# gusye1234/recad

Hardware: AMD Instinct MI355X
Metric: BPR train interactions/sec + full-catalog top-K scorings/sec, LightGCN ml1m dim=64 (higher is better)
Workload: dtype f32

## Files before the change

include/recad_hip.h:

```cpp
#ifndef RECAD_HIP_H
#define RECAD_HIP_H
#include <stdint.h>

#ifdef __cplusplus
extern "C" {
#endif

#define RK_ABI_VERSION 9
#define RK_OK 0
#define RK_EINVAL (-22)
#define RK_EHIP (-5)
#define RK_ENOMEM (-12)

#define RK_LOSS_PARTIALS 256

int rk_abi_version(void);
const char *rk_last_error(void);
int rk_device_info(char *name, int32_t name_len, int32_t *cu_count);

int rk_coo_to_csr(int32_t n_rows, int64_t nnz, const int64_t *coo_row, const int64_t *coo_col,
                  const float *coo_val, int32_t *rowptr , int32_t *col ,
                  float *val , void *stream);

typedef struct rk_schedule *rk_schedule_t;
// ... 139 lines not shown
    int32_t panel_rows;
    int32_t panel_ntw;
    int32_t panel_safe;
    int32_t nb, n_items, dim, K, n_targets;
    int32_t ld_scores;
    int32_t reserved[2];
    int64_t scratch_floats;
} rk_score_plan;
int rk_score_topk_plan(int32_t nb, int32_t n_items, int32_t dim, int32_t K, int32_t n_targets, const rk_score_plan *request ,
                       rk_score_plan *out);
int rk_score_topk(int32_t dim, const float *utab, int32_t nb, const int32_t *user_ids, const float *itab,
                  int32_t n_items, const float *ubias, const float *ibias, float mean,
                  const int32_t *seen_ptr, const int32_t *seen_idx, int32_t K, int32_t *top_ids,
                  float *top_scores, const int32_t *targets, int32_t n_targets, float *target_score,
                  int32_t *target_rank, const rk_score_plan *plan, float *scratch, void *stream);

int rk_mf_train_epoch(int32_t n_users, int32_t n_items, int32_t dim, float *user_emb, float *item_emb,
                      float *user_bias, float *item_bias, float mean, float *m, float *v, float *grads,
                      const int64_t *users, const int64_t *items, const int64_t *labels, int64_t n,
                      int32_t batch, int32_t adam_t0, float lr, float beta1, float beta2, float eps,
                      float *loss_partials, int32_t apply_update, float dropout, uint64_t drop_seed, void *stream);

int rk_bpr_sample(int32_t n_users, int32_t n_items, const int32_t *pos_ptr, const int32_t *pos_idx,
                  int64_t n_draws, uint64_t seed, int64_t *users, int64_t *pos, int64_t *neg, int32_t *valid,
                  void *stream);

int rk_pointwise_sample(int32_t n_users, int32_t n_items, const int32_t *train_ptr, const int32_t *train_idx,
                        int64_t n_edges, int32_t negative_ratio, uint64_t seed, int64_t *users, int64_t *items,
                        int64_t *labels, void *stream);

// ... 152 lines not shown
```

recad_amd/_lib.py:

```python
import ctypes as C
import os

import torch

_HERE = os.path.dirname(os.path.abspath(__file__))
LIB_PATH = os.path.join(_HERE, "lib", "librecad_hip.so")
RK_LOSS_PARTIALS = 256
RK_MAX_GRAPH_STEPS = 64
ABI_VERSION = 9
RK_LDS_SYNC_WORDS = 2560
RK_PCA_GRAM_BLOCKS = 256


class HipLibraryMissing(RuntimeError):
    pass


class HipCallError(RuntimeError):
    pass


class LdsInfo(C.Structure):

    _fields_ = [
# ... 137 lines not shown
    "rk_bpr_rows_ordered": [_I32, _I32, _F, _P, _P, _P, _P, _P, _P, _P, _I32, _P, _P, _P],
    "rk_lightgcn_create": [C.POINTER(LightGCNDesc), C.POINTER(_P)],
    "rk_lightgcn_destroy": [_P],
    "rk_lightgcn_sync_status": [_P, C.POINTER(_I32), _P],
    "rk_lightgcn_propagate": [_P, _P],
    "rk_lightgcn_propagate_dropout": [_P, C.c_uint64, _P],
    "rk_lightgcn_train_epoch": [_P, _P, _P, _P, _I64, _I32, _I32, _P, _I32, _I32, _P],
    "rk_lightgcn_prepare": [_P, _I64, _I32, _I32, _I32, _P],
    "rk_lightgcn_set_deterministic": [_P, _I32],
    "rk_pair_scores": [_I32, _P, _P, _P, _P, _F, _P, _P, _I64, _P, _F, C.c_uint64, _P],
    "rk_score_matrix": [_I32, _P, _I32, _P, _P, _I32, _P, _P, _F, _F, C.c_uint64, _P, _P],
    "rk_adam_step": [_I64, _P, _P, _P, _P, _I32, _F, _F, _F, _F, _P],
    "rk_adam_step_dev": [_I64, _P, _P, _P, _P, _P, _F, _F, _F, _P],
    "rk_score_topk_plan": [_I32, _I32, _I32, _I32, _I32, C.POINTER(ScorePlan), C.POINTER(ScorePlan)],
    "rk_score_topk": [_I32, _P, _I32, _P, _P, _I32, _P, _P, _F, _P, _P, _I32, _P, _P, _P, _I32, _P, _P, C.POINTER(ScorePlan), _P, _P],
    "rk_bpr_sample": [_I32, _I32, _P, _P, _I64, C.c_uint64, _P, _P, _P, _P, _P],
    "rk_pointwise_sample": [_I32, _I32, _P, _P, _I64, _I32, C.c_uint64, _P, _P, _P, _P],
    "rk_topk_rows": [_P, _I32, _I32, _P, _P, _P, _I32, _P, _P, _P, _I32, _P, _P, _P],
    "rk_hit_counts": [_P, _I64, _I32, _P, _I32, _P, _P],
    "rk_eligible_users": [_I32, _P, _P, _P, _I32, _P, _P, _P, _P],
    "rk_pred_shift": [_P, _P, _I64, _P, _P],
    "rk_users_rating": [_I32, _P, _I32, _P, _P, _I32, _P, _P],
    "rk_ncf_forward": [C.POINTER(NCFDesc), _P, _P, _P, _I32, _I64, _P, _P],
    "rk_ncf_train_epoch": [C.POINTER(NCFDesc), _P, _P, _P, _I64, _I32, _I32, _P, _I32, _P],
    "rk_mf_train_epoch": [_I32, _I32, _I32, _P, _P, _P, _P, _F, _P, _P, _P, _P, _P, _P, _I64, _I32, _I32, _F, _F, _F,
                          _F, _P, _I32, _F, C.c_uint64, _P],
    "rk_pca_transpose": [_I32, _I32, _P, _P, _P, _P, _P, _P, _P],
    "rk_pca_col_scale": [_I32, _I32, _P, _P, _P, _P, _P],
    "rk_pca_spmm": [_I32, _P, _P, _P, _P, _P, _I32, _P, _P, _P],
    "rk_pca_sq_spmv": [_I32, _I32, _P, _P, _P, _P, _I32, _I32, _P, _P, _P],
# ... 91 lines not shown
```

recad_amd/csrc/gemm.h:

```cpp
#pragma once
#include <stdlib.h>
#include <type_traits>

#include "common.h"

typedef float f32x16 __attribute__((ext_vector_type(16)));

struct GemmArgs {
    int M, N, K;
    const float *A; long long a_rs, a_cs;
    const int *a_ridx;
    int a_rmod, a_roff;
    const float *acc_init; int ld_init, init_base;
    const float *B; long long b_rs, b_cs;
    float *C; int ldc;
    const float *col_bias;
    const float *row_bias;
    float const_add;
    int relu;
    int sigmoid;
    unsigned drop_thresh24;
    float drop_scale;
    unsigned long long drop_seed;
    const float *mask; int ldmask;
    float *sk_part; long long sk_stride;
    int split_k;
};

static constexpr int kGK = 32, kGLd = kGK + 1;
template <int BT> constexpr int gemm_lds_bytes(int nbuf) { return nbuf * 2 * BT * kGLd * (int)sizeof(float); }

template <int BT> struct TileRegs { float v[BT / 8]; };

template <int BT>
__device__ __forceinline__ int tile_mode(const float *src, int n_rows, int n_k, int r0, int k0, long long rs, long long cs,
                                         bool gathered = false)
{
    const bool full = (r0 + BT <= n_rows) && (k0 + kGK <= n_k);
    if (!full) return 0;
    if (cs == 1 && (rs & 3) == 0 && ((uintptr_t)src & 15) == 0) return 1;
    if (!gathered && rs == 1 && (cs & 3) == 0 && ((uintptr_t)src & 15) == 0) return 2;
    return 0;
// ... 77 lines not shown
template <int BT, int NBUF, int MINW, bool GATHER = false, bool PLAIN = false>
static __global__ __launch_bounds__(256, MINW) void gemm_f32_kernel(const GemmArgs g, const int tiles_per_block)
{
    constexpr int kGT = BT, TA = BT / 64, WS = BT / 2;
    extern __shared__ __attribute__((aligned(16))) float smem[];
    auto tileA = [&](int buf) { return reinterpret_cast<float (*)[kGLd]>(smem + (size_t)buf * 2 * kGT * kGLd); };
    auto tileB = [&](int buf) { return reinterpret_cast<float (*)[kGLd]>(smem + (size_t)buf * 2 * kGT * kGLd + kGT * kGLd); };
    const int lane = threadIdx.x & 63, w = threadIdx.x >> 6;
    const int wr = w >> 1, wc = w & 1;
    const int gx = (g.N + kGT - 1) / kGT, gy = (g.M + kGT - 1) / kGT, nwg = gx * gy;
    int bid = blockIdx.x;
    {
        const int nb = gridDim.x, q = nb / 8, r = nb % 8, xcd = bid % 8;
        bid = (xcd < r ? xcd * (q + 1) : r * (q + 1) + (xcd - r) * q) + bid / 8;
    }
    const int t_begin = bid * tiles_per_block, t_end = min(nwg, t_begin + tiles_per_block);
    if (t_begin >= t_end) return;
    f32x16 acc[TA][TA];
#pragma unroll
    for (int i = 0; i < TA; ++i)
#pragma unroll
        for (int j = 0; j < TA; ++j)
#pragma unroll
            for (int r = 0; r < 16; ++r) acc[i][j][r] = 0.f;
    const int lr = lane & 31, lk = lane >> 5;
    const int all_chunks = (g.K + kGK - 1) / kGK;
    const int splits = g.split_k > 1 ? g.split_k : 1;
    const int per = (all_chunks + splits - 1) / splits;
    const int c_lo = (int)blockIdx.y * per, c_hi = min(all_chunks, c_lo + per);
    if (c_lo >= c_hi) return;
// ... 399 lines not shown
#define GEMM_STAMP(it, i) do { } while (0)
#endif
template <int MA, int MB, bool PLAIN = false, bool GROUPED = false>
static __global__ __launch_bounds__(256) __attribute__((amdgpu_waves_per_eu(2, 2))) void gemm_f32_wide_kernel(const GemmArgs g, const int gx, const int gy)
{
    extern __shared__ __attribute__((aligned(16))) float dsm[];
    float *sA = dsm, *sB = dsm + wide_floats<MA>();
    const int lane = threadIdx.x & 63, w = threadIdx.x >> 6, tid = threadIdx.x;
    const int wr = w >> 1, wc = w & 1;
    int bid = blockIdx.x;
    const int nb = gridDim.x;
    {
        const int q = nb / 8, r = nb % 8, xcd = bid % 8;
        bid = (xcd < r ? xcd * (q + 1) : r * (q + 1) + (xcd - r) * q) + bid / 8;
    }
    const int n_tiles = gx * gy;
    const int t_begin = (int)((long long)bid * n_tiles / nb), t_end = (int)((long long)(bid + 1) * n_tiles / nb);
    if (t_begin >= t_end) return;
    const int n_chunks = g.K / kWK, total = (t_end - t_begin) * n_chunks;
    f32x4 acc[4][4];
    const int l16 = lane & 15, lq = lane >> 4;
    long long ra[8], rb[8];
    int m0, n0, m1, n1;
    auto row_offsets = [&](int mt, int nt) {
#pragma unroll
        for (int p = 0; p < 8; ++p) {
            const int m = min(mt + p * 16 + (tid >> 4), g.M - 1);
            ra[p] = (long long)(g.a_ridx ? g.a_ridx[m] : g.a_rmod ? (m + g.a_roff) % g.a_rmod : m) * g.a_rs;
            rb[p] = (long long)min(nt + p * 16 + (tid >> 4), g.N - 1) * g.b_rs;
        }
// ... 189 lines not shown
        GEMM_STAMP(it, 6);
    }
}

inline hipError_t gemm_f32_launch(const GemmArgs &g, hipStream_t s)
{
    static RkPerDeviceOnce attr_once;
    static const int variant = RK_TUNE_INT("RK_GEMM_VARIANT", 0);
    int attr_dev;
    if (attr_once.need(&attr_dev)) {
        hipError_t e = hipFuncSetAttribute(reinterpret_cast<const void *>(gemm_f32_kernel<128, 2, 2>),
                                           hipFuncAttributeMaxDynamicSharedMemorySize, gemm_lds_bytes<128>(2));
        if (e != hipSuccess) return e;
        attr_once.done(attr_dev);
    }
    const int nwg128 = ((g.N + 127) / 128) * ((g.M + 127) / 128);
    if ((nwg128 < 384 || (g.split_k > 1 && g.sk_part)) && variant != 3 && !g.a_ridx && !g.a_rmod) {
        const int nwg = ((g.N + 63) / 64) * ((g.M + 63) / 64);
        GemmArgs g2 = g;
        const int splits = g2.split_k = gemm_effective_splits(g.K, g.split_k);
        const int chunks = (g.K + kGK - 1) / kGK, per = (chunks + splits - 1) / splits;
        static const int no_deep = RK_TUNE_INT("RK_GEMM_NO_DEEP", 0);
        static const int deep_min_k = RK_TUNE_INT("RK_GEMM_DEEP_MINK", 128);
        const int fa = deep_form(g.A, g.a_rs, g.a_cs), fb = deep_form(g.B, g.b_rs, g.b_cs);
        const bool deep = !no_deep && variant != 4 && fa && fb && !(fa == 2 && fb == 1) && g.M % 64 == 0 && g.N % 64 == 0 && g.K % kDK == 0 && per % 4 == 0 &&
                          per * kGK >= deep_min_k;
        if (variant == 4) hipLaunchKernelGGL((gemm_f32_kernel<64, 1, 4>), dim3(nwg, splits), dim3(256), gemm_lds_bytes<64>(1), s, g2, 1);
        else if (deep) {
            static const int no_half = RK_TUNE_INT("RK_GEMM_NO_HALF", 0);
            const bool half = nwg * splits < 256 && !no_half;
// ... 43 lines not shown
                    if (e != hipSuccess) return e;
                }
                wide_attr.done(wide_attr_dev);
            }
            int gx = (Ni + 127) / 128, gy = (g.M + 127) / 128;
            const size_t lds = (size_t)(wide_floats<1>() + (fb == 1 ? wide_floats<1>() : wide_floats<2>())) * sizeof(float);
            void *params[3] = {const_cast<GemmArgs *>(&g), &gx, &gy};
            hipError_t e = hipLaunchKernel(fn[fb == 2 ? 1 : plain_w ? (c_lines ? 3 : 2) : 0], dim3(std::min(gx * gy, wide_wgs)), dim3(256), params, lds, s);
            if (e != hipSuccess) return e;
            if (Ni < g.N) {
                GemmArgs e1 = g;
                e1.N = g.N - Ni; e1.B = g.B + (long long)Ni * g.b_rs; e1.C = g.C + Ni;
                if (g.col_bias) e1.col_bias = g.col_bias + Ni;
                if (g.mask) e1.mask = g.mask + Ni;
                if (g.acc_init) e1.acc_init = g.acc_init + Ni;
                e = gemm_f32_launch(e1, s);
                if (e != hipSuccess) return e;
            }
            return hipSuccess;
        }
    }
    int tpb = (g.K <= 64) ? nwg128 / 1024 : 1;
    static const int tpb_env = RK_TUNE_INT("RK_GEMM_TPB", 0);
    if (tpb_env > 0) tpb = tpb_env;
    tpb = tpb < 1 ? 1 : (tpb > 64 ? 64 : tpb);
    const dim3 grid((nwg128 + tpb - 1) / tpb);
    const bool plain = !g.row_bias && !g.col_bias && !g.relu && !g.mask && !g.sigmoid && !g.drop_thresh24;
    if (g.a_ridx && plain && !g.acc_init) hipLaunchKernelGGL((gemm_f32_kernel<128, 1, 3, true, true>), grid, dim3(256), gemm_lds_bytes<128>(1), s, g, tpb);
    else if (g.a_ridx || g.a_rmod) hipLaunchKernelGGL((gemm_f32_kernel<128, 1, 3, true, false>), grid, dim3(256), gemm_lds_bytes<128>(1), s, g, tpb);
    else if (variant == 1) hipLaunchKernelGGL((gemm_f32_kernel<128, 2, 2>), grid, dim3(256), gemm_lds_bytes<128>(2), s, g, tpb);
// ... 4 lines not shown
```

recad_amd/csrc/score_topk.hip:

```cpp
#include <algorithm>
#include <climits>

#include "gemm.h"
#include "score_panel.h"

static constexpr int kMaxK = 256;
static constexpr int kTopkNT = 256;
static constexpr int kInPassTargets = 4;

__device__ __forceinline__ void find_bin(const int *hist, int need, int tid, int *out)
{
    if (tid < 64) {
        const int4 v = *reinterpret_cast<const int4 *>(hist + 4 * tid);
        const int own = v.x + v.y + v.z + v.w;
        int inc = own;
#pragma unroll
        for (int o = 1; o < 64; o <<= 1) {
            const int n = __shfl_down(inc, o, 64);
            if (tid + o < 64) inc += n;
        }
        const int above = inc - own;
        if (above < need && need <= above + own) {
            int cum = above, bin = 4 * tid + 3, h = v.w;
            if (need > cum + h) { cum += h; bin = 4 * tid + 2; h = v.z; }
            if (need > cum + h) { cum += h; bin = 4 * tid + 1; h = v.y; }
            if (need > cum + h) { cum += h; bin = 4 * tid; h = v.x; }
            out[0] = bin; out[1] = need - cum; out[2] = cum + h;
        }
    }
    __syncthreads();
}

template <bool LDS_ROW>
__global__ __launch_bounds__(kTopkNT) void topk_rows_kernel(float *__restrict__ scores, long long ld, int n_items, const int *__restrict__ user_ids,
                                                            const int *__restrict__ seen_ptr, const int *__restrict__ seen_idx, int K,
                                                            int *__restrict__ top_ids, float *__restrict__ top_scores,
                                                            const int *__restrict__ targets, int n_targets,
                                                            float *__restrict__ target_score, int *__restrict__ target_rank)
{
    constexpr int NT = kTopkNT, NW = NT / 64;
    __shared__ __attribute__((aligned(16))) int hist[256];
    __shared__ __attribute__((aligned(16))) int hist2[256];
    __shared__ unsigned long long sel[kMaxK];
    __shared__ int sh_i[8];
    __shared__ int wtot[NW];
    __shared__ int tcount[kInPassTargets][NW];
    extern __shared__ __attribute__((aligned(16))) unsigned lds_keys[];
    const int tid = threadIdx.x, lane = tid & 63, w = tid >> 6;
    const int b = blockIdx.x;
    float *grow = scores + (size_t)b * (size_t)ld;
    auto key_at = [&](int i) -> unsigned { return LDS_ROW ? lds_keys[i] : score_key(grow[i]); };
    auto for_keys = [&](auto f) {
        if (LDS_ROW) {
// ... 89 lines not shown
            for (int t = 0; t < kInPassTargets; ++t)
                tc[t] += (k != 0u && i != tgt[t] && (k > tkey[t] || (k == tkey[t] && i < tgt[t]))) ? 1 : 0;
        });
#pragma unroll
        for (int t = 0; t < kInPassTargets; ++t) {
            const int c = (int)wave_sum((float)tc[t]);
            if (lane == 0) tcount[t][w] = c;
        }
    }
    if (mx != 0u) atomicAdd(&hist[mx >> 24], 1);
    __syncthreads();
    if (tid < n_in) {
        int tot = 0;
        for (int q = 0; q < NW; ++q) tot += tcount[tid][q];
        target_rank[(size_t)b * n_targets + tid] = tot;
    }
    for (int t = kInPassTargets; t < n_targets; ++t) {
        const int tg = targets[t];
        const unsigned kt = score_key(target_score[(size_t)b * n_targets + t]);
        int c = 0;
        for (int i = tid; i < n_items; i += NT) {
            const unsigned k = key_at(i);
            c += (k != 0u && i != tg && (k > kt || (k == kt && i < tg))) ? 1 : 0;
        }
        c = (int)wave_sum((float)c);
        __syncthreads();
        if (lane == 0) wtot[w] = c;
        __syncthreads();
        if (tid == 0) {
            int tot = 0;
            for (int q = 0; q < NW; ++q) tot += wtot[q];
            target_rank[(size_t)b * n_targets + t] = tot;
        }
    }

    unsigned cthr = 1u;
    find_bin(hist, K, tid, sh_i);
    if (sh_i[0] >= 0) {
        const unsigned d1 = (unsigned)sh_i[0];
        const int need1 = sh_i[1];
        if (mx != 0u && (mx >> 24) == d1) atomicAdd(&hist2[(mx >> 16) & 255u], 1);
        __syncthreads();
        find_bin(hist2, need1, tid, sh_i);
        cthr = max((d1 << 24) | ((unsigned)sh_i[0] << 16), 1u);
    }

    for_keys([&](int i, unsigned k) {
// ... 99 lines not shown
__device__ __forceinline__ void wave_lds_sync() { __builtin_amdgcn_fence(__ATOMIC_ACQ_REL, "workgroup"); __builtin_amdgcn_wave_barrier(); }
__device__ __forceinline__ int wave_sum_i(int v)
{
#pragma unroll
    for (int o = 32; o > 0; o >>= 1) v += __shfl_xor(v, o, 64);
    return v;
}
__device__ __forceinline__ int wave_incl_scan_i(int v, int lane)
{
#pragma unroll
    for (int o = 1; o < 64; o <<= 1) {
        const int n = __shfl_up(v, o, 64);
        if (lane >= o) v += n;
    }
    return v;
}
__device__ __forceinline__ unsigned score_key_sel(float s, bool excluded) { return excluded ? 0u : score_key(s); }
__device__ __forceinline__ void count_lt(int &c, unsigned a, unsigned b) { asm("v_cmp_lt_u32_e32 vcc, %1, %2\n\tv_addc_co_u32_e32 %0, vcc, 0, %0, vcc" : "+v"(c) : "s"(a), "v"(b) : "vcc"); }
__device__ __forceinline__ void count_le(int &c, unsigned a, unsigned b) { asm("v_cmp_le_u32_e32 vcc, %1, %2\n\tv_addc_co_u32_e32 %0, vcc, 0, %0, vcc" : "+v"(c) : "s"(a), "v"(b) : "vcc"); }
__device__ __forceinline__ void count_eq(int &c, unsigned a, unsigned b) { asm("v_cmp_eq_u32_e32 vcc, %1, %2\n\tv_addc_co_u32_e32 %0, vcc, 0, %0, vcc" : "+v"(c) : "s"(a), "v"(b) : "vcc"); }
static constexpr unsigned kKeyValid = 0x00800000u;
__device__ __forceinline__ unsigned score_key_raw(float s, unsigned ones)
{
    const unsigned u = __float_as_uint(s + 0.0f) | ones;
    return u ^ ((unsigned)((int)u >> 31) | 0x80000000u);
}

#ifndef TOPK_STAMP
#define TOPK_STAMP(i) do { } while (0)
#endif
#ifndef TOPK_WAVES_EU
#define TOPK_WAVES_EU(NQ) (NQ <= 58 ? 6 : NQ <= 72 ? 5 : 4), 8
#endif
#ifndef TOPK_WAVE_WG
#define TOPK_WAVE_WG 4
#endif
template <int NQ>
__global__ __launch_bounds__(64 * TOPK_WAVE_WG) __attribute__((amdgpu_waves_per_eu(TOPK_WAVES_EU(NQ)))) void topk_wave_kernel(
    const float *__restrict__ scores, long long ld, int nb, int n_items, const int *__restrict__ user_ids, const int *__restrict__ seen_ptr,
    const int *__restrict__ seen_idx, int K, int *__restrict__ top_ids, float *__restrict__ top_scores, const int *__restrict__ targets,
    int n_targets, float *__restrict__ target_score, int *__restrict__ target_rank)
{
    constexpr int NW = (NQ + 31) / 32;
    __shared__ unsigned bm_all[TOPK_WAVE_WG][NW * 64];
    __shared__ unsigned long long sel_all[TOPK_WAVE_WG][kMaxK + 4];
    const int lane = threadIdx.x & 63, w = __builtin_amdgcn_readfirstlane(threadIdx.x >> 6);
    const int b = (int)blockIdx.x * TOPK_WAVE_WG + w;
    if (b >= nb) return;
    TOPK_STAMP(0);
    unsigned *bm = bm_all[w];
    unsigned long long *sel = sel_all[w];
    unsigned *sel32 = reinterpret_cast<unsigned *>(sel_all[w]);
    const int hi = opaque(1);
    auto sel_put = [&](int slot, unsigned not_id, unsigned k) { sel32[2 * slot] = not_id; sel32[2 * slot + hi] = k; };
    const unsigned sel_base = (unsigned)reinterpret_cast<unsigned long long>(sel32);
    auto sel_put_at = [&](unsigned addr, unsigned not_id, unsigned k) {
// ... 51 lines not shown
            const int packed = wave_sum_i(c_gt + (c_eq << 16));
            int cnt = packed & 0xffff;
            const int n_eq = packed >> 16;
            const int self = (unsigned)tg < (unsigned)(NQ * 64) && !((bm[(tg >> 11) * 64 + (tg & 63)] >> ((tg >> 6) & 31)) & 1u) ? 1 : 0;
            if (n_eq > self && kt0 != 0u) {
                int ce = 0;
                const int lane_here = opaque(lane);
#pragma unroll
                for (int q = 0; q < NQ; ++q) {
                    ce += (key[q] == kt && lane_here + 64 * q < tg) ? 1 : 0;
                    if ((q & 7) == 7) __builtin_amdgcn_sched_barrier(0);
                }
                cnt += wave_sum_i(ce);
            }
            if (lane == 0) target_rank[(size_t)b * n_targets + t] = cnt;
        }
        TOPK_STAMP(4);
        unsigned m[4] = {0u, 0u, 0u, 0u};
#pragma unroll
        for (int q = 0; q < NQ; q += 8)
#pragma unroll
            for (int j = 0; j < 4; ++j) {
                if (q + 4 + j < NQ) m[j] = max(max(m[j], key[q + j]), key[q + 4 + j]);
                else if (q + j < NQ) m[j] = max(m[j], key[q + j]);
            }
        auto count_ge = [&](unsigned x) -> int {
            int c = 0;
#pragma unroll
            for (int j = 0; j < 4; ++j) c += __popcll(__ballot(m[j] >= x));
            return c;
// ... 51 lines not shown
            }
            const int n_gt = T == 0xffffffffu ? 0 : compact(T + 1u);
            const int need = K - n_gt;
            int before = 0;
#pragma unroll
            for (int q = 0; q < NQ; ++q) {
                const unsigned long long eq = __ballot(key[q] == T);
                const int pos = before + (int)__builtin_amdgcn_mbcnt_hi((unsigned)(eq >> 32), __builtin_amdgcn_mbcnt_lo((unsigned)eq, 0u));
                if (key[q] == T && pos < need) sel_put(n_gt + pos, ~(unsigned)lane - scalar_here(64 * q), T);
                before += __popcll(eq);
            }
            n_sel = K;
        }
        n_sel = __builtin_amdgcn_readfirstlane(n_sel);
        if (lane < 4) sel[n_sel + lane] = 0ULL;
        wave_lds_sync();
        TOPK_STAMP(6);
        unsigned long long mine[4];
        int rk[4] = {0, 0, 0, 0};
#pragma unroll
        for (int e = 0; e < 4; ++e) mine[e] = lane + 64 * e < n_sel ? sel[lane + 64 * e] : ~0ULL;
        auto rank_all = [&](auto ne) {
            constexpr int NE = decltype(ne)::value;
#pragma clang loop unroll(disable)
            for (int j = 0; j < n_sel; j += 4) {
                unsigned long long c[4];
#pragma unroll
                for (int i = 0; i < 4; ++i) c[i] = sel[j + i];
#pragma unroll
                for (int i = 0; i < 4; ++i)
// ... 15 lines not shown
            float sc = -INFINITY;
            if (k < n_sel) {
                const unsigned long long c = sel[k];
                id = (int)(~(unsigned)c);
                sc = key_score((unsigned)(c >> 32));
            }
            top_ids[(size_t)b * K + k] = id;
            top_scores[(size_t)b * K + k] = sc;
        }
        TOPK_STAMP(8);
    }
}

extern "C" int rk_topk_rows_impl(float *scores, long long ld, int nb, int n_items, const int *user_ids, const int *seen_ptr,
                                 const int *seen_idx, int K, int *top_ids, float *top_scores, const int *targets,
                                 int n_targets, float *target_score, int *target_rank, hipStream_t s)
{
    if (K <= 0 || K > kMaxK) RK_FAIL(RK_EINVAL, "top-K: K must be in [1,%d]", kMaxK);
    if (n_targets < 0 || n_targets > 256 || (n_targets > 0 && (!targets || !target_score || !target_rank)))
        RK_FAIL(RK_EINVAL, "top-K: bad targets");
    if (ld < n_items) RK_FAIL(RK_EINVAL, "top-K: row stride %lld < n_items %d", ld, n_items);
    static const int no_wave = RK_TUNE_INT("RK_TOPK_NO_WAVE", 0);
    if (!no_wave && n_items <= 96 * 64) {
        const int nq = (n_items + 63) / 64;
        const dim3 grid((nb + TOPK_WAVE_WG - 1) / TOPK_WAVE_WG), block(64 * TOPK_WAVE_WG);
#define RK_TOPK_WAVE(NQ)                                                                                                              \
    hipLaunchKernelGGL((topk_wave_kernel<NQ>), grid, block, 0, s, scores, ld, nb, n_items, user_ids, seen_ptr, seen_idx, K, top_ids, \
                       top_scores, targets, n_targets, target_score, target_rank)
        if (nq <= 16) RK_TOPK_WAVE(16);
        else if (nq <= 32) RK_TOPK_WAVE(32);
        else if (nq <= 48) RK_TOPK_WAVE(48);
        else if (nq <= 58) RK_TOPK_WAVE(58);
        else if (nq <= 64) RK_TOPK_WAVE(64);
        else if (nq <= 80) RK_TOPK_WAVE(80);
        else if (nq <= 88) RK_TOPK_WAVE(88);
        else RK_TOPK_WAVE(96);
#undef RK_TOPK_WAVE
        RK_CHECK_LAUNCH();
        return RK_OK;
    }
    const size_t row_bytes = ((size_t)n_items * sizeof(float) + 15) & ~(size_t)15;
    static const size_t lds_row_max = (size_t)RK_TUNE_INT("RK_TOPK_LDS_KB", 40) * 1024;
    if (row_bytes <= lds_row_max) {
        static RkPerDeviceOnce attr_once;
        int attr_dev;
        if (attr_once.need(&attr_dev)) {
            RK_HIP(hipFuncSetAttribute(reinterpret_cast<const void *>(topk_rows_kernel<true>),
                                       hipFuncAttributeMaxDynamicSharedMemorySize, 64 * 1024));
            attr_once.done(attr_dev);
        }
        hipLaunchKernelGGL((topk_rows_kernel<true>), dim3(nb), dim3(kTopkNT), row_bytes, s, scores, ld, n_items, user_ids, seen_ptr, seen_idx,
                           K, top_ids, top_scores, targets, n_targets, target_score, target_rank);
    } else {
        hipLaunchKernelGGL((topk_rows_kernel<false>), dim3(nb), dim3(kTopkNT), 0, s, scores, ld, n_items, user_ids, seen_ptr, seen_idx, K,
                           top_ids, top_scores, targets, n_targets, target_score, target_rank);
    }
    RK_CHECK_LAUNCH();
    return RK_OK;
}

static inline long long score_ld(int n_items) { return ((long long)n_items + 31) & ~31LL; }

static bool panel_by_default(int nb, int n_items, int dim, int K, int n_targets)
{
    if (!pan_supported(n_items, dim, K, n_targets)) return false;
    if (n_targets > 1 && dim > 64) return false;
    if (nb >= 8192) return n_items >= kPanDefaultMinItems / 2;
    return n_items >= kPanDefaultMinItems && nb >= 4096 && dim <= 64;
}

RK_EXPORT int rk_score_topk_plan(int32_t nb, int32_t n_items, int32_t dim, int32_t K, int32_t n_targets, const rk_score_plan *request,
                                 rk_score_plan *out)
{
// ... 11 lines not shown
    if (pl.path == RK_SCORE_PANEL) {
        const int rows = request ? request->panel_rows : 0, ntw = request ? request->panel_ntw : 0;
        if ((rows != 0 && rows != 16 && rows != 32) || (ntw != 0 && ntw != 8 && ntw != 15)) RK_FAIL(RK_EINVAL, "rk_score_topk_plan: panel_rows in {16, 32}, panel_ntw in {8, 15}");
        pl.panel_ntw = ntw ? ntw : pan_ntw(n_items);
        pl.panel_rows = pl.panel_ntw == 8 ? 16 : (rows ? rows : pan_rows(nb, n_items, dim, n_targets));
        pl.panel_safe = request && request->panel_safe ? 1 : 0;
        pl.scratch_floats = (int64_t)pan_scratch_floats(n_items, dim);
    } else {
        pl.ld_scores = (int32_t)score_ld(n_items);
        pl.scratch_floats = (int64_t)nb * pl.ld_scores;
    }
    *out = pl;
    return RK_OK;
}

RK_EXPORT int rk_score_topk(int32_t dim, const float *utab, int32_t nb, const int32_t *user_ids, const float *itab,
                            int32_t n_items, const float *ubias, const float *ibias, float mean,
                            const int32_t *seen_ptr, const int32_t *seen_idx, int32_t K, int32_t *top_ids,
                            float *top_scores, const int32_t *targets, int32_t n_targets, float *target_score,
                            int32_t *target_rank, const rk_score_plan *plan, float *scratch, void *stream)
{
    if (nb <= 0) return RK_OK;
    if (dim <= 0 || n_items <= 0 || !utab || !itab || !user_ids || !seen_ptr || !seen_idx || !scratch || !top_ids || !top_scores || !plan)
        RK_FAIL(RK_EINVAL, "rk_score_topk: bad arguments");
    if ((ubias == nullptr) != (ibias == nullptr)) RK_FAIL(RK_EINVAL, "rk_score_topk: give both biases or neither");
    if (K <= 0 || K > kMaxK) RK_FAIL(RK_EINVAL, "top-K: K must be in [1,%d]", kMaxK);
    if (n_targets < 0 || n_targets > 256 || (n_targets > 0 && (!targets || !target_score || !target_rank)))
        RK_FAIL(RK_EINVAL, "top-K: bad targets");
    if (plan->n_items != n_items || plan->dim != dim || plan->K != K || plan->n_targets != n_targets || nb > plan->nb)
        RK_FAIL(RK_EINVAL, "rk_score_topk: the plan was made for another request (rk_score_topk_plan)");
    hipStream_t s = (hipStream_t)stream;
    if (plan->path == RK_SCORE_PANEL) {
        if (!pan_supported(n_items, dim, K, n_targets)) RK_FAIL(RK_EINVAL, "rk_score_topk: the panel form does not take this request");
        if (reinterpret_cast<uintptr_t>(scratch) & 15) RK_FAIL(RK_EINVAL, "rk_score_topk: scratch must be 16-byte aligned (panel form)");
        PanArgs a;
        memset(&a, 0, sizeof(a));
        a.nb = nb; a.n_items = n_items; a.d = dim; a.K = K;
        a.utab = utab; a.user_ids = user_ids; a.itab = itab; a.ubias = ubias; a.ibias = ibias; a.mean = mean;
        a.seen_ptr = seen_ptr; a.seen_idx = seen_idx; a.targets = targets; a.n_targets = n_targets;
        a.top_ids = top_ids; a.top_scores = top_scores; a.target_score = target_score; a.target_rank = target_rank;
        RK_HIP(score_panel_launch(a, scratch, s, plan->panel_rows, plan->panel_ntw, plan->panel_safe));
        return RK_OK;
    }
    if (plan->path != RK_SCORE_GEMM) RK_FAIL(RK_EINVAL, "rk_score_topk: plan->path %d", plan->path);
    GemmArgs g;
    memset(&g, 0, sizeof(g));
    g.M = nb; g.N = n_items; g.K = dim;
    g.A = utab; g.a_rs = dim; g.a_cs = 1; g.a_ridx = user_ids;
    g.B = itab; g.b_rs = dim; g.b_cs = 1;
    if (plan->ld_scores != (int32_t)score_ld(n_items)) RK_FAIL(RK_EINVAL, "rk_score_topk: plan->ld_scores %d (rk_score_topk_plan sets it)", plan->ld_scores);
    g.C = scratch; g.ldc = plan->ld_scores;
    g.row_bias = ubias; g.col_bias = ibias; g.const_add = mean;
    RK_HIP(gemm_f32_launch(g, s));
    return rk_topk_rows_impl(scratch, plan->ld_scores, nb, n_items, user_ids, seen_ptr, seen_idx, K, top_ids, top_scores, targets, n_targets,
                             target_score, target_rank, s);
}

__global__ __launch_bounds__(1024) void hit_counts_kernel(const int *__restrict__ rank, long long n, int T, const int *__restrict__ ks,
                                                          int nk, int *__restrict__ counts, int use_atomics)
{
    constexpr int KG = 4;
    __shared__ int wtot[KG][16];
    const int tid = threadIdx.x, lane = tid & 63, w = tid >> 6;
    for (int t = 0; t < T; ++t)
        for (int q0 = 0; q0 < nk; q0 += KG) {
            int kk[KG], c[KG];
#pragma unroll
            for (int q = 0; q < KG; ++q) { kk[q] = q0 + q < nk ? ks[q0 + q] : INT_MIN; c[q] = 0; }
            for (long long b = (long long)blockIdx.x * 1024 + tid; b < n; b += (long long)gridDim.x * 1024) {
                const int r = rank[b * T + t];
// ... 4 lines not shown
            for (int q = 0; q < KG; ++q) {
                const int s = (int)wave_sum((float)c[q]);
                if (lane == 0) wtot[q][w] = s;
            }
            __syncthreads();
            if (tid < KG && q0 + tid < nk) {
                int tot = 0;
                for (int i = 0; i < 16; ++i) tot += wtot[tid][i];
                if (use_atomics) atomicAdd(&counts[t * nk + q0 + tid], tot);
                else counts[t * nk + q0 + tid] = tot;
            }
            __syncthreads();
        }
}

RK_EXPORT int rk_hit_counts(const int32_t *target_rank, int64_t n, int32_t n_targets, const int32_t *ks, int32_t nk,
                            int32_t *counts, void *stream)
{
    if (n_targets <= 0 || nk <= 0) return RK_OK;
    if (n < 0 || !target_rank || !ks || !counts) RK_FAIL(RK_EINVAL, "rk_hit_counts: bad arguments");
    hipStream_t s = (hipStream_t)stream;
    const int grid = (int)std::max<long long>(1, std::min<long long>(64, (n + 16383) / 16384));
    if (grid > 1) RK_HIP(rk_zero_async(counts, sizeof(int32_t) * (size_t)n_targets * nk, s));
    hipLaunchKernelGGL(hit_counts_kernel, dim3(grid), dim3(1024), 0, s, target_rank, (long long)n, n_targets, ks, nk, counts, grid > 1);
    RK_CHECK_LAUNCH();
    return RK_OK;
}

__global__ void eligible_flags_kernel(int n_users, const int *__restrict__ ptr, const int *__restrict__ idx,
                                      const int *__restrict__ targets, int n_targets, int *__restrict__ flags)
{
    for (int u = blockIdx.x * blockDim.x + threadIdx.x; u < n_users; u += gridDim.x * blockDim.x) {
        const int b = ptr[u], e = ptr[u + 1];
        int ok = e > b ? 1 : 0;
        for (int t = 0; t < n_targets && ok; ++t) {
            const int x = targets[t];
            int lo = b, hi = e;
            while (lo < hi) { const int mid = (lo + hi) >> 1; if (idx[mid] < x) lo = mid + 1; else hi = mid; }
            if (lo < e && idx[lo] == x) ok = 0;
// ... 108 lines not shown
```

recad_amd/evaluate.py:

```python
import ctypes as C

import numpy as np
import torch

from . import _lib


def score_plan(nb, n_items, dim, K, n_targets, request=None):
    req = _lib.ScorePlan()
    if request:
        req.path = {"auto": _lib.RK_SCORE_AUTO, "gemm": _lib.RK_SCORE_GEMM, "panel": _lib.RK_SCORE_PANEL}[request.get("path", "auto")]
        req.panel_rows, req.panel_ntw = int(request.get("panel_rows", 0)), int(request.get("panel_ntw", 0))
        req.panel_safe = 1 if request.get("panel_safe") else 0
    out = _lib.ScorePlan()
    _lib.check(_lib.lib().rk_score_topk_plan(int(nb), int(n_items), int(dim), int(K), int(n_targets), C.byref(req) if request else None,
                                             C.byref(out)), "rk_score_topk_plan")
    return out


SCORE_REQUEST = None


def full_catalog_topk(victim, user_ids, seen_ptr, seen_idx, targets, K=100, chunk=4096, to_host=True, request=None, extra_scratch_floats=0):
    _lib.require_gpu()
# ... 123 lines not shown
            if tuple(tabs[1].shape) != (self.plan.n_items, self.plan.dim):
                raise RuntimeError("EvalSession: the victim's item table changed shape; build a new session")
            self._static_tabs, self._static_key = tabs, key
            self._graph, self._graph_key = None, None

    def _launch(self):
        v, L, plan = self.victim, _lib.lib(), self.plan
        utab, itab, ubias, ibias, mean = self._static_tabs if self._static_tabs is not None else v.scoring_tables()
        utab, itab = utab.contiguous(), itab.contiguous()
        if ubias is not None:
            ubias, ibias = ubias.contiguous().view(-1), ibias.contiguous().view(-1)
        n_items, d = itab.shape
        st = _lib.stream_ptr()
        for s in range(0, self.n, self.chunk):
            e = min(self.n, s + self.chunk)
            _lib.check(L.rk_score_topk(
                d, _lib.ptr(utab), e - s, _lib.ptr(self.users[s:e]), _lib.ptr(itab), n_items, _lib.ptr(ubias), _lib.ptr(ibias), float(mean),
                _lib.ptr(self.seen_ptr), _lib.ptr(self.seen_idx), self.K, _lib.ptr(self.top_ids[s:e]), _lib.ptr(self.top_scores[s:e]),
                _lib.ptr(self.targets), self.T, _lib.ptr(self.tscore[s:e]), _lib.ptr(self.trank[s:e]), C.byref(plan), _lib.ptr(self.scratch), st),
                "rk_score_topk")
        if self.T and self.n:
            _lib.check(L.rk_hit_counts(_lib.ptr(self.trank), self.n, self.T, _lib.ptr(self.ks), len(self.topks), _lib.ptr(self.counts), st), "rk_hit_counts")

    def run(self):
        self._runs += 1
        self._refresh_static()
        key = (getattr(self.victim, "_handle_key", None), self._static_key)
        if self.want_graph and self._graph is not None and self._graph_key == key:
            self._graph.replay()
        else:
            self._launch()
            if self.want_graph and self._runs >= 2 and (self._graph is None or self._graph_key != key):
                try:
                    torch.cuda.synchronize()
                    g = torch.cuda.CUDAGraph()
                    with torch.cuda.graph(g):
                        self._launch()
# ... 69 lines not shown
```

Measured before the change: 15.44 million.

## Fuse hit-count accumulation into top-K kernels and zero counters inside GEMM

Adds rk_score_topk_hr, which updates the hit@k counters with atomics directly inside the top-K kernels, and zeroes the counter array from the first GEMM block on the first chunk. This removes the separate rk_hit_counts launch and the memset launch from the evaluation session. The cost is atomic contention on a small counter array. It also relies on stream ordering so the zeroing in the GEMM finishes before the top-K kernel increments the counters. An extra LDS waitcnt is added before a wave sync.

```diff
diff --git a/include/recad_hip.h b/include/recad_hip.h
--- a/include/recad_hip.h
+++ b/include/recad_hip.h
@@ -177,6 +177,12 @@
                   const int32_t *seen_ptr, const int32_t *seen_idx, int32_t K, int32_t *top_ids,
                   float *top_scores, const int32_t *targets, int32_t n_targets, float *target_score,
                   int32_t *target_rank, const rk_score_plan *plan, float *scratch, void *stream);
+int rk_score_topk_hr(int32_t dim, const float *utab, int32_t nb, const int32_t *user_ids, const float *itab,
+                     int32_t n_items, const float *ubias, const float *ibias, float mean,
+                     const int32_t *seen_ptr, const int32_t *seen_idx, int32_t K, int32_t *top_ids,
+                     float *top_scores, const int32_t *targets, int32_t n_targets, float *target_score,
+                     int32_t *target_rank, const rk_score_plan *plan, float *scratch, const int32_t *ks, int32_t nk,
+                     int32_t *counts, int32_t first_chunk, void *stream);
 
 int rk_mf_train_epoch(int32_t n_users, int32_t n_items, int32_t dim, float *user_emb, float *item_emb,
                       float *user_bias, float *item_bias, float mean, float *m, float *v, float *grads,
diff --git a/recad_amd/_lib.py b/recad_amd/_lib.py
--- a/recad_amd/_lib.py
+++ b/recad_amd/_lib.py
@@ -175,6 +175,8 @@
     "rk_adam_step_dev": [_I64, _P, _P, _P, _P, _P, _F, _F, _F, _P],
     "rk_score_topk_plan": [_I32, _I32, _I32, _I32, _I32, C.POINTER(ScorePlan), C.POINTER(ScorePlan)],
     "rk_score_topk": [_I32, _P, _I32, _P, _P, _I32, _P, _P, _F, _P, _P, _I32, _P, _P, _P, _I32, _P, _P, C.POINTER(ScorePlan), _P, _P],
+    "rk_score_topk_hr": [_I32, _P, _I32, _P, _P, _I32, _P, _P, _F, _P, _P, _I32, _P, _P, _P, _I32, _P, _P, C.POINTER(ScorePlan), _P, _P, _I32, _P,
+                         _I32, _P],
     "rk_bpr_sample": [_I32, _I32, _P, _P, _I64, C.c_uint64, _P, _P, _P, _P, _P],
     "rk_pointwise_sample": [_I32, _I32, _P, _P, _I64, _I32, C.c_uint64, _P, _P, _P, _P],
     "rk_topk_rows": [_P, _I32, _I32, _P, _P, _P, _I32, _P, _P, _P, _I32, _P, _P, _P],
diff --git a/recad_amd/csrc/gemm.h b/recad_amd/csrc/gemm.h
--- a/recad_amd/csrc/gemm.h
+++ b/recad_amd/csrc/gemm.h
@@ -25,7 +25,14 @@
     const float *mask; int ldmask;
     float *sk_part; long long sk_stride;
     int split_k;
+    int *zero_words; int n_zero;
 };
+
+__device__ __forceinline__ void gemm_zero_words(const GemmArgs &g)
+{
+    if (g.n_zero > 0 && blockIdx.x == 0 && blockIdx.y == 0)
+        for (int i = threadIdx.x; i < g.n_zero; i += 256) g.zero_words[i] = 0;
+}
 
 static constexpr int kGK = 32, kGLd = kGK + 1;
 template <int BT> constexpr int gemm_lds_bytes(int nbuf) { return nbuf * 2 * BT * kGLd * (int)sizeof(float); }
@@ -133,6 +140,7 @@
         const int nb = gridDim.x, q = nb / 8, r = nb % 8, xcd = bid % 8;
         bid = (xcd < r ? xcd * (q + 1) : r * (q + 1) + (xcd - r) * q) + bid / 8;
     }
+    if (GATHER) gemm_zero_words(g);
     const int t_begin = bid * tiles_per_block, t_end = min(nwg, t_begin + tiles_per_block);
     if (t_begin >= t_end) return;
     f32x16 acc[TA][TA];
@@ -562,6 +570,7 @@
         const int q = nb / 8, r = nb % 8, xcd = bid % 8;
         bid = (xcd < r ? xcd * (q + 1) : r * (q + 1) + (xcd - r) * q) + bid / 8;
     }
+    gemm_zero_words(g);
     const int n_tiles = gx * gy;
     const int t_begin = (int)((long long)bid * n_tiles / nb), t_end = (int)((long long)(bid + 1) * n_tiles / nb);
     if (t_begin >= t_end) return;
@@ -781,6 +790,7 @@
         if (e != hipSuccess) return e;
         attr_once.done(attr_dev);
     }
+    if (g.n_zero > 0 && (!g.a_ridx || !g.zero_words)) return hipErrorInvalidValue;
     const int nwg128 = ((g.N + 127) / 128) * ((g.M + 127) / 128);
     if ((nwg128 < 384 || (g.split_k > 1 && g.sk_part)) && variant != 3 && !g.a_ridx && !g.a_rmod) {
         const int nwg = ((g.N + 63) / 64) * ((g.M + 63) / 64);
@@ -854,6 +864,7 @@
                 if (g.col_bias) e1.col_bias = g.col_bias + Ni;
                 if (g.mask) e1.mask = g.mask + Ni;
                 if (g.acc_init) e1.acc_init = g.acc_init + Ni;
+                e1.n_zero = 0;
                 e = gemm_f32_launch(e1, s);
                 if (e != hipSuccess) return e;
             }
diff --git a/recad_amd/csrc/score_topk.hip b/recad_amd/csrc/score_topk.hip
--- a/recad_amd/csrc/score_topk.hip
+++ b/recad_amd/csrc/score_topk.hip
@@ -31,12 +31,15 @@
     __syncthreads();
 }
 
+__device__ __forceinline__ void hr_add(int *__restrict__ counts, const int *__restrict__ ks, int nk, int t, int rank, int first, int step);
+
 template <bool LDS_ROW>
 __global__ __launch_bounds__(kTopkNT) void topk_rows_kernel(float *__restrict__ scores, long long ld, int n_items, const int *__restrict__ user_ids,
                                                             const int *__restrict__ seen_ptr, const int *__restrict__ seen_idx, int K,
                                                             int *__restrict__ top_ids, float *__restrict__ top_scores,
                                                             const int *__restrict__ targets, int n_targets,
-                                                            float *__restrict__ target_score, int *__restrict__ target_rank)
+                                                            float *__restrict__ target_score, int *__restrict__ target_rank,
+                                                            const int *__restrict__ ks, int nk, int *__restrict__ hr_counts)
 {
     constexpr int NT = kTopkNT, NW = NT / 64;
     __shared__ __attribute__((aligned(16))) int hist[256];
@@ -156,6 +159,7 @@
         int tot = 0;
         for (int q = 0; q < NW; ++q) tot += tcount[tid][q];
         target_rank[(size_t)b * n_targets + tid] = tot;
+        hr_add(hr_counts, ks, nk, tid, tot, 0, 1);
     }
     for (int t = kInPassTargets; t < n_targets; ++t) {
         const int tg = targets[t];
@@ -173,6 +177,7 @@
             int tot = 0;
             for (int q = 0; q < NW; ++q) tot += wtot[q];
             target_rank[(size_t)b * n_targets + t] = tot;
+            hr_add(hr_counts, ks, nk, t, tot, 0, 1);
         }
     }
 
@@ -302,6 +307,12 @@
         if (lane >= o) v += n;
     }
     return v;
+}
+__device__ __forceinline__ void hr_add(int *__restrict__ counts, const int *__restrict__ ks, int nk, int t, int rank, int first, int step)
+{
+    if (!counts) return;
+    for (int q = first; q < nk; q += step)
+        if (rank < ks[q]) atomicAdd(&counts[t * nk + q], 1);
 }
 __device__ __forceinline__ unsigned score_key_sel(float s, bool excluded) { return excluded ? 0u : score_key(s); }
 __device__ __forceinline__ void count_lt(int &c, unsigned a, unsigned b) { asm("v_cmp_lt_u32_e32 vcc, %1, %2\n\tv_addc_co_u32_e32 %0, vcc, 0, %0, vcc" : "+v"(c) : "s"(a), "v"(b) : "vcc"); }
@@ -327,7 +338,8 @@
 __global__ __launch_bounds__(64 * TOPK_WAVE_WG) __attribute__((amdgpu_waves_per_eu(TOPK_WAVES_EU(NQ)))) void topk_wave_kernel(
     const float *__restrict__ scores, long long ld, int nb, int n_items, const int *__restrict__ user_ids, const int *__restrict__ seen_ptr,
     const int *__restrict__ seen_idx, int K, int *__restrict__ top_ids, float *__restrict__ top_scores, const int *__restrict__ targets,
-    int n_targets, float *__restrict__ target_score, int *__restrict__ target_rank)
+    int n_targets, float *__restrict__ target_score, int *__restrict__ target_rank, const int *__restrict__ ks, int nk,
+    int *__restrict__ hr_counts)
 {
     constexpr int NW = (NQ + 31) / 32;
     __shared__ unsigned bm_all[TOPK_WAVE_WG][NW * 64];
@@ -409,6 +421,7 @@
                 cnt += wave_sum_i(ce);
             }
             if (lane == 0) target_rank[(size_t)b * n_targets + t] = cnt;
+            hr_add(hr_counts, ks, nk, t, cnt, lane, 64);
         }
         TOPK_STAMP(4);
         unsigned m[4] = {0u, 0u, 0u, 0u};
@@ -490,6 +503,7 @@
         }
         n_sel = __builtin_amdgcn_readfirstlane(n_sel);
         if (lane < 4) sel[n_sel + lane] = 0ULL;
+        asm volatile("s_waitcnt lgkmcnt(0)" : : : "memory");
         wave_lds_sync();
         TOPK_STAMP(6);
         unsigned long long mine[4];
@@ -535,7 +549,11 @@
 
 extern "C" int rk_topk_rows_impl(float *scores, long long ld, int nb, int n_items, const int *user_ids, const int *seen_ptr,
                                  const int *seen_idx, int K, int *top_ids, float *top_scores, const int *targets,
-                                 int n_targets, float *target_score, int *target_rank, hipStream_t s)
+                                 int n_targets, float *target_score, int *target_rank, hipStream_t s);
+
+static int topk_rows_launch(float *scores, long long ld, int nb, int n_items, const int *user_ids, const int *seen_ptr,
+                            const int *seen_idx, int K, int *top_ids, float *top_scores, const int *targets,
+                            int n_targets, float *target_score, int *target_rank, const int *ks, int nk, int *hr_counts, hipStream_t s)
 {
     if (K <= 0 || K > kMaxK) RK_FAIL(RK_EINVAL, "top-K: K must be in [1,%d]", kMaxK);
     if (n_targets < 0 || n_targets > 256 || (n_targets > 0 && (!targets || !target_score || !target_rank)))
@@ -547,7 +565,7 @@
         const dim3 grid((nb + TOPK_WAVE_WG - 1) / TOPK_WAVE_WG), block(64 * TOPK_WAVE_WG);
 #define RK_TOPK_WAVE(NQ)                                                                                                              \
     hipLaunchKernelGGL((topk_wave_kernel<NQ>), grid, block, 0, s, scores, ld, nb, n_items, user_ids, seen_ptr, seen_idx, K, top_ids, \
-                       top_scores, targets, n_targets, target_score, target_rank)
+                       top_scores, targets, n_targets, target_score, target_rank, ks, nk, hr_counts)
         if (nq <= 16) RK_TOPK_WAVE(16);
         else if (nq <= 32) RK_TOPK_WAVE(32);
         else if (nq <= 48) RK_TOPK_WAVE(48);
@@ -571,13 +589,21 @@
             attr_once.done(attr_dev);
         }
         hipLaunchKernelGGL((topk_rows_kernel<true>), dim3(nb), dim3(kTopkNT), row_bytes, s, scores, ld, n_items, user_ids, seen_ptr, seen_idx,
-                           K, top_ids, top_scores, targets, n_targets, target_score, target_rank);
+                           K, top_ids, top_scores, targets, n_targets, target_score, target_rank, ks, nk, hr_counts);
     } else {
         hipLaunchKernelGGL((topk_rows_kernel<false>), dim3(nb), dim3(kTopkNT), 0, s, scores, ld, n_items, user_ids, seen_ptr, seen_idx, K,
-                           top_ids, top_scores, targets, n_targets, target_score, target_rank);
+                           top_ids, top_scores, targets, n_targets, target_score, target_rank, ks, nk, hr_counts);
     }
     RK_CHECK_LAUNCH();
     return RK_OK;
+}
+
+extern "C" int rk_topk_rows_impl(float *scores, long long ld, int nb, int n_items, const int *user_ids, const int *seen_ptr,
+                                 const int *seen_idx, int K, int *top_ids, float *top_scores, const int *targets,
+                                 int n_targets, float *target_score, int *target_rank, hipStream_t s)
+{
+    return topk_rows_launch(scores, ld, nb, n_items, user_ids, seen_ptr, seen_idx, K, top_ids, top_scores, targets, n_targets, target_score,
+                            target_rank, nullptr, 0, nullptr, s);
 }
 
 static inline long long score_ld(int n_items) { return ((long long)n_items + 31) & ~31LL; }
@@ -619,13 +645,20 @@
     return RK_OK;
 }
 
-RK_EXPORT int rk_score_topk(int32_t dim, const float *utab, int32_t nb, const int32_t *user_ids, const float *itab,
-                            int32_t n_items, const float *ubias, const float *ibias, float mean,
-                            const int32_t *seen_ptr, const int32_t *seen_idx, int32_t K, int32_t *top_ids,
-                            float *top_scores, const int32_t *targets, int32_t n_targets, float *target_score,
-                            int32_t *target_rank, const rk_score_plan *plan, float *scratch, void *stream)
-{
-    if (nb <= 0) return RK_OK;
+static void hit_counts_launch(const int *rank, long long n, int T, const int *ks, int nk, int *counts, int grid, int use_atomics, hipStream_t s);
+
+static int score_topk_run(int32_t dim, const float *utab, int32_t nb, const int32_t *user_ids, const float *itab,
+                          int32_t n_items, const float *ubias, const float *ibias, float mean,
+                          const int32_t *seen_ptr, const int32_t *seen_idx, int32_t K, int32_t *top_ids,
+                          float *top_scores, const int32_t *targets, int32_t n_targets, float *target_score,
+                          int32_t *target_rank, const rk_score_plan *plan, float *scratch, const int32_t *ks, int32_t nk,
+                          int32_t *counts, int32_t first_chunk, void *stream)
+{
+    const int n_counts = counts ? n_targets * nk : 0;
+    if (nb <= 0) {
+        if (n_counts > 0 && first_chunk) RK_HIP(rk_zero_async(counts, sizeof(int32_t) * (size_t)n_counts, (hipStream_t)stream));
+        return RK_OK;
+    }
     if (dim <= 0 || n_items <= 0 || !utab || !itab || !user_ids || !seen_ptr || !seen_idx || !scratch || !top_ids || !top_scores || !plan)
         RK_FAIL(RK_EINVAL, "rk_score_topk: bad arguments");
     if ((ubias == nullptr) != (ibias == nullptr)) RK_FAIL(RK_EINVAL, "rk_score_topk: give both biases or neither");
@@ -645,6 +678,11 @@
         a.seen_ptr = seen_ptr; a.seen_idx = seen_idx; a.targets = targets; a.n_targets = n_targets;
         a.top_ids = top_ids; a.top_scores = top_scores; a.target_score = target_score; a.target_rank = target_rank;
         RK_HIP(score_panel_launch(a, scratch, s, plan->panel_rows, plan->panel_ntw, plan->panel_safe));
+        if (n_counts > 0) {
+            if (first_chunk) RK_HIP(rk_zero_async(counts, sizeof(int32_t) * (size_t)n_counts, s));
+            hit_counts_launch(target_rank, nb, n_targets, ks, nk, counts, (int)std::max(1, std::min(64, (nb + 16383) / 16384)), 1, s);
+            RK_CHECK_LAUNCH();
+        }
         return RK_OK;
     }
     if (plan->path != RK_SCORE_GEMM) RK_FAIL(RK_EINVAL, "rk_score_topk: plan->path %d", plan->path);
@@ -656,9 +694,34 @@
     if (plan->ld_scores != (int32_t)score_ld(n_items)) RK_FAIL(RK_EINVAL, "rk_score_topk: plan->ld_scores %d (rk_score_topk_plan sets it)", plan->ld_scores);
     g.C = scratch; g.ldc = plan->ld_scores;
     g.row_bias = ubias; g.col_bias = ibias; g.const_add = mean;
+    if (n_counts > 0 && first_chunk) { g.zero_words = counts; g.n_zero = n_counts; }
     RK_HIP(gemm_f32_launch(g, s));
-    return rk_topk_rows_impl(scratch, plan->ld_scores, nb, n_items, user_ids, seen_ptr, seen_idx, K, top_ids, top_scores, targets, n_targets,
-                             target_score, target_rank, s);
+    return topk_rows_launch(scratch, plan->ld_scores, nb, n_items, user_ids, seen_ptr, seen_idx, K, top_ids, top_scores, targets, n_targets,
+                            target_score, target_rank, ks, nk, n_counts > 0 ? counts : nullptr, s);
+}
+
+RK_EXPORT int rk_score_topk(int32_t dim, const float *utab, int32_t nb, const int32_t *user_ids, const float *itab,
+                            int32_t n_items, const float *ubias, const float *ibias, float mean,
+                            const int32_t *seen_ptr, const int32_t *seen_idx, int32_t K, int32_t *top_ids,
+                            float *top_scores, const int32_t *targets, int32_t n_targets, float *target_score,
+                            int32_t *target_rank, const rk_score_plan *plan, float *scratch, void *stream)
+{
+    return score_topk_run(dim, utab, nb, user_ids, itab, n_items, ubias, ibias, mean, seen_ptr, seen_idx, K, top_ids, top_scores, targets,
+                          n_targets, target_score, target_rank, plan, scratch, nullptr, 0, nullptr, 0, stream);
+}
+
+RK_EXPORT int rk_score_topk_hr(int32_t dim, const float *utab, int32_t nb, const int32_t *user_ids, const float *itab,
+                               int32_t n_items, const float *ubias, const float *ibias, float mean,
+                               const int32_t *seen_ptr, const int32_t *seen_idx, int32_t K, int32_t *top_ids,
+                               float *top_scores, const int32_t *targets, int32_t n_targets, float *target_score,
+                               int32_t *target_rank, const rk_score_plan *plan, float *scratch, const int32_t *ks, int32_t nk,
+                               int32_t *counts, int32_t first_chunk, void *stream)
+{
+    if (nk < 0 || (n_targets > 0 && nk > 0 && (!ks || !counts))) RK_FAIL(RK_EINVAL, "rk_score_topk_hr: bad counters");
+    const bool want = n_targets > 0 && nk > 0;
+    return score_topk_run(dim, utab, nb, user_ids, itab, n_items, ubias, ibias, mean, seen_ptr, seen_idx, K, top_ids, top_scores, targets,
+                          n_targets, target_score, target_rank, plan, scratch, want ? ks : nullptr, want ? nk : 0, want ? counts : nullptr,
+                          first_chunk, stream);
 }
 
 __global__ __launch_bounds__(1024) void hit_counts_kernel(const int *__restrict__ rank, long long n, int T, const int *__restrict__ ks,
@@ -693,6 +756,11 @@
         }
 }
 
+static void hit_counts_launch(const int *rank, long long n, int T, const int *ks, int nk, int *counts, int grid, int use_atomics, hipStream_t s)
+{
+    hipLaunchKernelGGL(hit_counts_kernel, dim3(grid), dim3(1024), 0, s, rank, n, T, ks, nk, counts, use_atomics);
+}
+
 RK_EXPORT int rk_hit_counts(const int32_t *target_rank, int64_t n, int32_t n_targets, const int32_t *ks, int32_t nk,
                             int32_t *counts, void *stream)
 {
@@ -701,7 +769,7 @@
     hipStream_t s = (hipStream_t)stream;
     const int grid = (int)std::max<long long>(1, std::min<long long>(64, (n + 16383) / 16384));
     if (grid > 1) RK_HIP(rk_zero_async(counts, sizeof(int32_t) * (size_t)n_targets * nk, s));
-    hipLaunchKernelGGL(hit_counts_kernel, dim3(grid), dim3(1024), 0, s, target_rank, (long long)n, n_targets, ks, nk, counts, grid > 1);
+    hit_counts_launch(target_rank, (long long)n, n_targets, ks, nk, counts, grid, grid > 1, s);
     RK_CHECK_LAUNCH();
     return RK_OK;
 }
diff --git a/recad_amd/evaluate.py b/recad_amd/evaluate.py
--- a/recad_amd/evaluate.py
+++ b/recad_amd/evaluate.py
@@ -161,13 +161,12 @@
         st = _lib.stream_ptr()
         for s in range(0, self.n, self.chunk):
             e = min(self.n, s + self.chunk)
-            _lib.check(L.rk_score_topk(
+            _lib.check(L.rk_score_topk_hr(
                 d, _lib.ptr(utab), e - s, _lib.ptr(self.users[s:e]), _lib.ptr(itab), n_items, _lib.ptr(ubias), _lib.ptr(ibias), float(mean),
                 _lib.ptr(self.seen_ptr), _lib.ptr(self.seen_idx), self.K, _lib.ptr(self.top_ids[s:e]), _lib.ptr(self.top_scores[s:e]),
-                _lib.ptr(self.targets), self.T, _lib.ptr(self.tscore[s:e]), _lib.ptr(self.trank[s:e]), C.byref(plan), _lib.ptr(self.scratch), st),
-                "rk_score_topk")
-        if self.T and self.n:
-            _lib.check(L.rk_hit_counts(_lib.ptr(self.trank), self.n, self.T, _lib.ptr(self.ks), len(self.topks), _lib.ptr(self.counts), st), "rk_hit_counts")
+                _lib.ptr(self.targets), self.T, _lib.ptr(self.tscore[s:e]), _lib.ptr(self.trank[s:e]), C.byref(plan), _lib.ptr(self.scratch),
+                _lib.ptr(self.ks), len(self.topks), _lib.ptr(self.counts), 1 if s == 0 else 0, st),
+                "rk_score_topk_hr")
 
     def run(self):
         self._runs += 1
```

Result: no change. 15.38 million (-0.4%).
